# PolyChord/PolyChordLite

Measured on AMD Instinct MI355X. Metric: likelihood evals/sec, 20D Gaussian nlive=2000, higher is better.
Workload: dtype f64; 1 GPU; configs[1]: 20-D Gaussian, nlive=2000, num_repeats=40, one full run per step; batch_chains=1000, parallelism=repeat-sharded x1, mode=one run at a time per GPU; R runs in step: roofline.in_step

## Files before the change

### polychordlite_amd/csrc/pc_contract.hip

```cpp
#include "pc_state.h"
#include "pc_launch.h"
#include <atomic>
#include <cstdlib>
#include <type_traits>

template <int NT>
__device__ __forceinline__ vk_t block_argmin(vk_t v, vk_t *scratch)
{
    v = wave_argmin(v);
    if (NT == 64) return v;
    const int wid = threadIdx.x >> 6;
    if ((threadIdx.x & 63) == 0) scratch[wid] = v;
    __syncthreads();
    vk_t r = scratch[0];
#pragma unroll
    for (int i = 1; i < NT / 64; ++i) r = vk_min(r, scratch[i]);
    __syncthreads();
    return r;
}

struct ConsumeShared {
    double *sL; int *sC; int *sP;
    double *cLogLp, *cLogXp, *cLogZp, *cLogZXp, *cLogZp2, *cLogZpXp, *cLseRef, *cLseSum, *cThr;
    int *cN, *cMinSlot; unsigned *cUid;
// ... 1138 lines not shown
#pragma unroll
                    for (int u = 0; u < 8; ++u) if (u < cnt) dst0[(size_t)idx[u] * nT + e] = v[u];
                }
            }
        }
        return;
    }
    for (int m = 0; m < (nr + 62) / 64; ++m) {
        const unsigned long long mask = S.plan[w].ph_mask[m];
        if (wv == 0 && ((mask >> lane) & 1ull)) {
            const int i = m * 64 + lane, dsti = base + __popcll(mask & ((1ull << lane) - 1ull));
            S.ph_logL[dsti] = S.baby_logL[(size_t)w * nr + i]; S.ph_cuid[dsti] = cuid;
            S.ph_uid[dsti] = ((unsigned long long)batch << 32) | (unsigned)(w * nr + i);
        }
        const unsigned long long mine = mask & (0xFFFFull << (16 * wv));
        const int before = __popcll(mask & ((1ull << (16 * wv)) - 1ull));
        wave_copy_masked(S.babies + ((size_t)w * nr + m * 64) * nT, mine, S.phantom + (size_t)(base + before) * nT, nT, lane);
        base += __popcll(mask);
    }
}
__global__ __launch_bounds__(64 * PC_APPLY_WAVES) void k_apply_dead_ph(PcState S, unsigned batch) { apply_dead_ph_body(S, batch); }
__global__ __launch_bounds__(64 * PC_APPLY_WAVES) void k_apply_dead_ph_many(const PcManyRec *__restrict__ R) { apply_dead_ph_body(pc_many_state(R, blockIdx.y), (unsigned)R[blockIdx.y].ia[PC_REC_I_BATCH]); }

__device__ __forceinline__ void apply_pool_body(const PcState &S, unsigned batch, int nchains)
{
    const PcCtl *ctl = S.ctl;
    const int lane = threadIdx.x & 63, nT = S.nT, nr = S.nr;
    const int item = (int)blockIdx.x * (int)(blockDim.x >> 6) + (int)(threadIdx.x >> 6);
    if (item >= nchains + S.Ncap) return;
    if (item < nchains) {
        const int w = ctl->seg_lo + item;
        if (w > ctl->seg_hi) return;
        const int di = S.plan[w].dead_idx, src = S.plan[w].dead_src;
        if (di >= 0 && src < 0) {
            const double *row = S.babies + ((size_t)(-src - 1) * nr + (nr - 1)) * nT;
            double *dst = S.dead + (size_t)di * nT;
            for (int e = lane; e < nT; e += 64) dst[e] = row[e];
            if (lane == 0) {
                S.dead_logw[di] = S.plan[w].logw; S.dead_postX[di] = S.plan[w].postX + log(S.plan[w].postXs); S.dead_postZ[di] = S.plan[w].postZ;
                S.dead_cuid[di] = S.plan[w].dead_cuid; S.dead_entry[di] = S.plan[-src - 1].contour;
            }
        }
        const int base = S.plan[w].ph_base;
        const unsigned cuid = S.plan[w].ph_cuid;
        const double Lg = S.plan[w].contour;
        for (int i = lane; i < nr; i += 64) {
            const double bl = S.baby_logL[(size_t)w * nr + i];
            S.ph_logL[base + i] = bl; S.ph_cuid[base + i] = ((i < nr - 1) && bl > Lg) ? cuid : PC_CUID_NONE;
            S.ph_uid[base + i] = ((unsigned long long)batch << 32) | (unsigned)(w * nr + i);
        }
        return;
    }
    const int slot = item - nchains;
    const int src = S.slot_src[slot], killer = S.slot_dead[slot];
    if (src < 0 && killer < 0) return;
    double *lrow = S.live + (size_t)slot * nT;
    if (killer >= 0) {
        const int di = S.plan[killer].dead_idx;
        double *dst = S.dead + (size_t)di * nT;
        for (int e = lane; e < nT; e += 64) dst[e] = lrow[e];
        if (lane == 0) {
            S.dead_logw[di] = S.plan[killer].logw; S.dead_postX[di] = S.plan[killer].postX + log(S.plan[killer].postXs); S.dead_postZ[di] = S.plan[killer].postZ;
            S.dead_cuid[di] = S.plan[killer].dead_cuid; S.dead_entry[di] = S.live_entry[slot];
        }
    }
    if (src >= 0) {
        const double *row = S.babies + ((size_t)src * nr + (nr - 1)) * nT;
        double v[4];
#pragma unroll
        for (int q = 0; q < 4; ++q) v[q] = (lane + 64 * q < nT) ? row[lane + 64 * q] : 0.0;
        for (int e = lane + 256; e < nT; e += 64) lrow[e] = row[e];
#pragma unroll
        for (int q = 0; q < 4; ++q) if (lane + 64 * q < nT) lrow[lane + 64 * q] = v[q];
    }
    if (lane == 0) { S.slot_src[slot] = -1; S.slot_dead[slot] = -1; if (src >= 0) S.live_entry[slot] = S.plan[src].contour; }
}
__global__ __launch_bounds__(256) void k_apply_pool(PcState S, unsigned batch, int nchains) { apply_pool_body(S, batch, nchains); }
__global__ __launch_bounds__(256) void k_apply_pool_many(const PcManyRec *R, int nchains) { apply_pool_body(pc_many_state(R, blockIdx.y), (unsigned)R[blockIdx.y].ia[PC_REC_I_BATCH], nchains); }


__device__ __forceinline__ void apply_live_body(const PcState &S)
{
    const int slot = blockIdx.x, lane = threadIdx.x, nT = S.nT, nr = S.nr;
    const int src = S.slot_src[slot];
    if (src < 0) return;
    const double *row = S.babies + ((size_t)src * nr + (nr - 1)) * nT;
    double *dst = S.live + (size_t)slot * nT;
    for (int e = lane; e < nT; e += 64) dst[e] = row[e];
    __syncthreads();
    if (lane == 0) { S.slot_src[slot] = -1; S.live_entry[slot] = S.plan[src].contour; }
}
__global__ __launch_bounds__(64) void k_apply_live(PcState S) { apply_live_body(S); }
__global__ __launch_bounds__(64) void k_apply_live_many(const PcManyRec *__restrict__ R) { apply_live_body(pc_many_state(R, blockIdx.y)); }

__global__ __launch_bounds__(256) void k_install_live(PcState S, const double *rows, int n)
{
    const int tid = threadIdx.x;
    __shared__ vk_t red[4];
    for (int s = tid; s < S.Ncap; s += 256) {
        if (s < n) {
            S.live_logL[s] = rows[(size_t)s * S.nT + S.l0]; S.live_cluster[s] = 0; S.live_pos[s] = s; S.live_entry[s] = S.logzero;
// ... 582 lines not shown
        const size_t sh = consume_lds(S, 1024, cache_x, 0, sgl);
        if (sh > 160 * 1024) return 1;
        pc_need_dyn_lds((const void *)k_consume<1024>, sh);
        hipLaunchKernelGGL((k_consume<1024>), dim3(1), dim3(1024), sh, st, *S, final_mode, cache_x, 0, sgl);
    } else {
        const int sgl = consume_slots_global(S, 64);
        int xr = S->Ncap;
        while (xr > 32 && consume_lds(S, 64, xr, 0, sgl) > 158 * 1024) xr = (xr + 1) / 2;
        const size_t sh = consume_lds(S, 64, xr, 0, sgl);
        if (sh > 160 * 1024) return 1;
        pc_need_dyn_lds((const void *)k_consume<64>, sh);
        hipLaunchKernelGGL((k_consume<64>), dim3(1), dim3(64), sh, st, *S, final_mode, xr, 0, sgl);
    }
    return 0;
}

extern "C" void pc_launch_apply(const PcState *S, unsigned batch, int nchains, hipStream_t st)
{
    if (S->pool) { hipLaunchKernelGGL(k_apply_pool, dim3((nchains + S->Ncap + 3) / 4), dim3(256), 0, st, *S, batch, nchains); return; }
    hipLaunchKernelGGL(k_apply_dead_ph, dim3(nchains), dim3(64 * PC_APPLY_WAVES), 0, st, *S, batch);
    hipLaunchKernelGGL(k_apply_live, dim3(S->Ncap), dim3(64), 0, st, *S);
}

extern "C" int pc_launch_apply_many(const PcState *S, const PcManyRec *dR, int R, unsigned batch, int nchains, hipStream_t st)
{
    if (!S->pool) {
        hipLaunchKernelGGL(k_apply_dead_ph_many, dim3(nchains, R), dim3(64 * PC_APPLY_WAVES), 0, st, dR);
        hipLaunchKernelGGL(k_apply_live_many, dim3(S->Ncap, R), dim3(64), 0, st, dR);
        return 0;
    }
    static const int wpg = std::getenv("PC_APPLY_WAVES") ? std::max(1, std::min(4, std::atoi(std::getenv("PC_APPLY_WAVES")))) : 4;
    hipLaunchKernelGGL(k_apply_pool_many, dim3((nchains + S->Ncap + wpg - 1) / wpg, R), dim3(64 * wpg), 0, st, dR, nchains);
    return 0;
}

extern "C" int pc_launch_clean_many(const PcManyRec *dR, int R, int nblk_max, hipStream_t st)
{
    if (nblk_max < 1) return 1;
    hipLaunchKernelGGL(k_clean_flag_many, dim3(nblk_max, R), dim3(256), 0, st, dR);
    hipLaunchKernelGGL(k_scan_blocks_many, dim3(1, R), dim3(256), 0, st, dR);
    hipLaunchKernelGGL(k_clean_scatter_many, dim3(nblk_max, R), dim3(256), 0, st, dR);
    return 0;
}

extern "C" void pc_launch_install_live(const PcState *S, const double *rows, int n, hipStream_t st)
{
// ... 195 lines not shown
```

### polychordlite_amd/csrc/pc_engine.hip

```cpp
#include "pc_state.h"
#include "pc_resume.h"
#include "pc_prior_table.h"
#include "pc_launch.h"
#include "pc_plan.h"
#include <cstdio>
#include <cstdlib>
#include <cstring>
#include <cstdarg>
#include <cstdint>
#include <new>
#include <cmath>
#include <vector>
#include <memory>
#include <string>
#include <chrono>
#include <algorithm>
#include <map>
#include <unordered_map>
#include <atomic>
#include <mutex>
#include <thread>
#include <functional>
#include <exception>
#include <ucontext.h>
// ... 292 lines not shown
    std::vector<int> cb_idx; std::vector<double> cb_c, cb_t, cb_p, cb_l;
    polychord_dumper_fn dumper = nullptr;
    pchip_update_fn on_update = nullptr; void *hook_user = nullptr;
    long ndiscarded = 0;
    bool resume_static = true; unsigned resume_batch0 = 0;
    bool nph_stale = false;
    std::vector<double> hm_dead, hm_logw; int hm_ndead = 0;
    std::vector<unsigned> hm_cuid;
    std::vector<double> pp_rows, pp_logpost; std::vector<unsigned> pp_cuid; std::vector<unsigned long long> pp_uid; int nd_last_update = 0;
    std::vector<unsigned> split_child, split_parent; std::vector<double> split_logfrac;
    std::vector<double> h_lo, h_hi;
    PcState S{};
    RunBlocks blocks;
    hipStream_t st = nullptr;
    hipStream_t st_copy = nullptr;
    bool st_copy_shared = false;
    hipStream_t st_side = nullptr;
    hipEvent_t ev_main = nullptr;
    static constexpr int RAW_RING = 4;
    struct RawSlot { hipEvent_t ready = nullptr, consumed = nullptr; unsigned batch = 0; int B = 0; bool valid = false, waited = false, used = false; int co_seq = 0; };
    RawSlot ring[RAW_RING];
    int raw_depth = 2;
    double *h_dead = nullptr; size_t h_dead_cap = 0, h_dead_copied = 0;
    PcCtl *h_ctl = nullptr;
    PcCtl *h_note = nullptr;
    unsigned note_seq = 0;
    hipEvent_t ev_apply = nullptr;
    double *raw_buf[RAW_RING] = {nullptr, nullptr, nullptr, nullptr};
    double *ph2 = nullptr, *phL2 = nullptr; unsigned *phC2 = nullptr; unsigned long long *phU2 = nullptr;
    unsigned char *keep = nullptr; int *blk = nullptr, *d_total = nullptr;
    double *psum = nullptr, *mean = nullptr, *pcov = nullptr; int *pcnt = nullptr, *count = nullptr;
    size_t cov_chunks_cap = 0;
    double *upd_part = nullptr, *upd_shift = nullptr; size_t upd_part_cap = 0;
    PcPriorTable ptab; bool have_ptab = false;
    double *d_lo = nullptr, *d_hi = nullptr, *d_invcovT = nullptr, *d_mean = nullptr, *d_src = nullptr;
    double *d_dynL = nullptr; int *d_dynN = nullptr; double *d_logn = nullptr;
    ClusterUpdate<Engine> clus{*this};
    Engine() = default; Engine(const Engine &) = delete; Engine &operator=(const Engine &) = delete;
    std::vector<int> sub_dims; int *c_subdims = nullptr;
    long nsplits = 0; int ncluster_peak = 1;
    bool src_terms = false;
    long path[PCHIP_PATH_COUNT] = {};
    Cohort::Note step_note;
    Timing tm;
    KTimer kt;
    int B = 0, dev = 0;
// ... 581 lines not shown

    PcLaunchTraits launch_traits() const { return PcLaunchTraits{pc_rtc_wanted(&S) != 0, src_terms, S.prior.kind >= PCHIP_PRIOR_TABLE}; }
    PcUpdateFacts update_facts(int nph) const { return PcUpdateFacts{nph > 0, pc_update_fused_ok(&S, h_ctl->ncluster) != 0, h_ctl->ncluster}; }

    void do_update(bool deferred = false)
    {
        tm.updates += deferred ? std::max(1, h_ctl->upd_marks) : 1;
        const bool seq_post = S.seq_mode && (cfg.posteriors || cfg.equals);
        if (plan.ctl == PC_CTL_EARLY) { const int st_keep = h_ctl->status; read_ctl(); h_ctl->status = st_keep; }
        if (!plan.hook_late) call_dumper();
        const int nph = S.pool ? (int)pool_cursor : h_ctl->nphantom;
        const PcUpdateChoice upd = pc_choose_update(plan, update_facts(nph));
        pc_count(path, upd);
        if (upd.kind == PC_UPDATE_FUSED) {
            const size_t need = (size_t)pc_update_fused_blocks(&S, nph) * pc_update_fused_entries(&S);
            if (need > upd_part_cap) { blocks.release(upd_part); upd_part_cap = 2 * need; upd_part = blocks.dev<double>(upd_part_cap); }
            if (!upd_shift) {
                upd_shift = blocks.dev<double>(S.D);
                std::vector<double> half(S.D, 0.5);
                HIPCHK(hipMemcpyAsync(upd_shift, half.data(), sizeof(double) * S.D, hipMemcpyHostToDevice, st));
                HIPCHK(hipStreamSynchronize(st));
            }
            hipEvent_t e0 = kt.begin(KT_CLEAN);
            (void)stage(rec_update(S, keep, blk, d_total, ph2, phL2, phC2, phU2, upd_part, upd_shift, co ? pc_update_fused_grid(&S, nph, deferred ? 1 : 0) : 0, deferred, nph));
            kt.end(KT_CLEAN, e0);
            if (upd.need_count) {
                std::vector<int> tot;
                fetch(tot, (const int *)d_total, 1);
                fetch_wait();
                const int total = tot[0];
                h_ctl->nphantom = total;
                if (seq_post) seq_consume((unsigned long long)(nph - total));
            } else nph_stale = true;
            if (!S.pool) { std::swap(S.phantom, ph2); std::swap(S.ph_logL, phL2); std::swap(S.ph_cuid, phC2); std::swap(S.ph_uid, phU2); }
            write_resume();
            return;
        }
        if (deferred) engine_fail(PC_RC_DEVICE, "deferred update without the fused update path");
        hipEvent_t e0 = kt.begin(KT_CLEAN);
        if (co && nph <= 0) { direct_op(); pc_launch_clean(&S, nph, keep, blk, d_total, ph2, phL2, phC2, phU2, nullptr, st); }
        else (void)stage(rec_compact(S, keep, blk, d_total, ph2, phL2, phC2, phU2, nph));
        kt.end(KT_CLEAN, e0);
        if (plan.hook_late) { collect_phantom_posteriors(nph); call_dumper(); }
        const bool need_count = upd.need_count, ctl_late = upd.ctl == PC_CTL_LATE;
        int total = nph;
        std::vector<int> tot, cn;
        if (need_count) {
// ... 438 lines not shown
        bool resumed = false;
        if (cfg.resume_read) {
            if (FILE *probe = std::fopen(cfg.resume_read, "r")) {
                std::fclose(probe);
                PcResume rs; std::string err;
                if (!pc_resume_read(cfg.resume_read, rs, err) || !import_resume(rs, err)) { std::fprintf(stderr, "polychord_hip: %s\n", err.c_str()); return 6; }
                resumed = true;
                int ntot = 0;
                for (int v : rs.nlive) ntot += v;
                if (ntot > cfg.nlive && rs.ncluster == 1) { pc_count(path, PcTrimLive{}); pc_launch_consume(&S, 2, 0, st); read_ctl(); ntot = cfg.nlive; }
                resume_static = (ntot == cfg.nlive);
                resume_batch0 = (unsigned)rs.ndead;
            }
        }
        if (!resumed) { if (callback_mode) generate_live_callback(); else generate_live(); }
        if (stop.load(std::memory_order_relaxed)) return 5;
        if (cb_auto_batch && !(cb_eval_seconds >= 0.0 && cb_eval_seconds < 2e-6)) { B = B_small; S.B = B; }
        r_t1 = clk::now();
        r_batch = resume_batch0;
        r_sort_valid = false;
        r_nursery_left = 0;
        make_plan();
        S.defer_update = plan.defer ? 1 : 0; S.pool = plan.pool ? 1 : 0;
        if (S.pool) {
            pool_cursor = h_ctl->nphantom;
            if (g_cap_phantoms.load() <= 0) {
                size_t free_b = 0, total_b = 0;
                (void)hipMemGetInfo(&free_b, &total_b);
                const double need = 2.0 * 2.0 * (double)S.Pcap * ((double)S.nT * 8.0 + 24.0);
                if (need < 0.4 * (double)free_b) grow_phantoms(2LL * S.Pcap);
            }
        }
        r_rc = 0;
        return -1;
    }

    void make_plan()
    {
        const int nprior0 = cfg.nprior <= 0 ? cfg.nlive : cfg.nprior;
        PcRunFacts f{};
        f.ablate = cfg.ablate; f.force_general = cfg.force_general;
        f.fixed_nlive = (cfg.n_nlives == 0) && (nprior0 >= cfg.nlive) && resume_static;
        f.par_fits = pc_par_fits(&S) != 0; f.fast_fits = pc_fast_fits(&S) != 0; f.fused_fits_one = pc_update_fused_ok(&S, 1) != 0;
        f.clustering = cfg.do_clustering != 0; f.boost = cfg.boost_posterior != 0.0;
        f.dumper = dumper != nullptr; f.on_update = on_update != nullptr; f.resume_write = cfg.resume_write != nullptr;
        f.seq_mode = S.seq_mode != 0; f.posteriors = cfg.posteriors || cfg.equals;
// ... 184 lines not shown
                sort_valid = false;
                if (ch.want_nn) { co->rec(rec_nn(S, nursery_left)); S.nn_valid = 1; }
                co->rec(rec_sort(S));
                co->rec(rec_consume_cl(S, h_ctl->ncluster > 64));
                break;
            case PC_CONTRACT_CL: case PC_CONTRACT_GENERAL: {
                sort_valid = false;
                if (co) co->flush();
                bool sorted_now = false;
                if (presorted) { HIPCHK(hipStreamWaitEvent(st, ev_presort_b, 0)); sorted_now = fresh_nursery; presorted = false; }
                if (ch.want_nn) {
                    if (!sorted_now) sorted_now = pc_launch_sort_live(&S, st) == 0;
                    pc_launch_nn_lists(&S, nursery_left, sorted_now ? 1 : 0, st);
                    S.nn_valid = 1;
                }
                if (ch.kind == PC_CONTRACT_CL) rc2 = (sorted_now ? 0 : pc_launch_sort_live(&S, st)) || pc_launch_consume_cl(&S, h_ctl->ncluster, st);
                else rc2 = pc_launch_consume(&S, 0, (h_ctl->ncluster > 1) ? 1 : 0, st);
                break;
            }
            }
            if (rc2) { std::fprintf(stderr, "polychord_hip: nlive too large for the LDS-resident contraction\n"); r_rc = 4; return false; }
            kt.end(KT_CONSUME, e2);
            hipEvent_t e3 = kt.begin(KT_APPLY);
            (void)stage(rec_apply(S, batch - 1, B));
            kt.end(KT_APPLY, e3);
            if (st_side) { RawSlot &rs = ring[batch % raw_depth]; if (rs.valid && rs.batch == batch && !rs.waited) { HIPCHK(hipStreamWaitEvent(st, rs.ready, 0)); rs.waited = true; } }
            r_fresh = fresh_nursery;
            ready_spins = 0;
        }
        return true;
    }

    bool finish_may_wait() const
    {
        const bool upd = h_ctl->status == PC_ST_UPDATE || (h_ctl->upd_pending && h_ctl->status == PC_ST_RUNNING);
        return upd && pc_choose_update(plan, update_facts(1)).may_wait;
    }
    bool round_finish()
    {
        unsigned &batch = r_batch; int &nursery_left = r_nursery_left; const bool fresh_nursery = r_fresh;
        (void)batch;
        {
            if (fresh_nursery && h_ctl->status == PC_ST_DONE && h_ctl->i_nursery == B) tm.batches--;
            nursery_left = h_ctl->i_nursery;
            tally_grades();
            tm.rounds++;
// ... 722 lines not shown
```

### polychordlite_amd/csrc/pc_launch.h

```cpp
#pragma once
#include "pc_state.h"
#include "../../include/polychord_hip.h"
#include <cstddef>

extern "C" int pc_rtc_source_sums(int id);
extern "C" long pc_rtc_source_quad(int id);

static inline size_t pc_quad_lds(const PcState *S)
{
    if (S->like.kind != PC_LIKE_SOURCE) return 0;
    const long n = pc_rtc_source_quad(S->src_id);
    return n > 0 ? sizeof(double) * 2 * (size_t)((n + 1) & ~1L) : 0;
}

static inline int pc_slice_phi_lds(const PcState *S)
{
    const size_t sh0 = sizeof(double) * ((size_t)S->D + S->nr) + 16, tb = sizeof(double) * (size_t)S->nr * (S->D + 1);
    const size_t sums = S->like.kind == PC_LIKE_SOURCE ? sizeof(double) * (size_t)S->nr * (size_t)pc_rtc_source_sums(S->src_id) : 0;
    return (S->nDer > 0 && sh0 + tb + sums + pc_quad_lds(S) <= 48 * 1024) ? 1 : 0;
}

extern "C" {

void pc_abi_set_last_error(const char *msg);
void pc_launch_slice_tick(const PcState *S, unsigned batch, int nchains, void *cs, double *x0s, int *decks, double *prop, const double *ev_logL,
                          const double *ev_theta, const double *ev_phi, int first, double *prop_host, int *need_host, hipStream_t st);
size_t pc_chain_state_size(void);
int pc_launch_killoff_cl(const PcState *S, int nc, hipStream_t st);
int pc_consume_cl_fits(const PcState *S, int nc);
int pc_consume_clp_fits(const PcState *S, int nc);
int pc_launch_consume_cl_many(const PcState *S, const PcManyRec *dR, int R, int wide, hipStream_t st);
int pc_launch_consume_cl(const PcState *S, int nc, hipStream_t st);
int pc_launch_knn_cluster_sub(const int *d_desc, int nb, int mmax, const double *Sm, const int *pool, int *knn, int *labels, int *out, hipStream_t st);
int pc_launch_knn_cluster_sub_many(const PcManyRec *dR, int R, int nb_max, int mmax, hipStream_t st);
void pc_launch_remap_chains(const PcState *S, const int *map, int nold, int n, hipStream_t st);
void pc_launch_shift_mats(const PcState *S, int p, int nc, hipStream_t st);
int pc_launch_knn_cluster_batch(const PcState *S, const int *h_desc, const int *d_desc, int nd, double *Sm, int *knn, int *labels, int *out, const int *dims, int ndims, hipStream_t st);
int pc_launch_knn_cluster_batch_dev(const PcState *S, const int *d_desc, int nd, int nmax, double *Sm, int *knn, int *labels, int *out, const int *dims, int ndims, hipStream_t st);
int pc_launch_knn_cluster_batch_many(const PcState *S, const PcManyRec *dR, int R, int nd_max, int nmax, int any_sub, hipStream_t st);
void pc_launch_rebuild(const PcState *S, int nc, hipStream_t st);
void pc_launch_ph_rehome(const PcState *S, int nph, int nc, const unsigned *old_uids, int nold_uids, int *counts, hipStream_t st);
void pc_launch_nn_lists(const PcState *S, int nleft, int use_rank, hipStream_t st);
int pc_launch_nn_lists_many(const PcState *S, const PcManyRec *dR, int R, int nleft_max, int use_rank, hipStream_t st);
int pc_launch_consume(const PcState *S, int final_mode, int wide, hipStream_t st);
void pc_launch_apply(const PcState *S, unsigned batch, int nchains, hipStream_t st);
int pc_launch_apply_many(const PcState *S, const PcManyRec *dR, int R, unsigned batch, int nchains, hipStream_t st);
int pc_launch_clean_many(const PcManyRec *dR, int R, int nblk_max, hipStream_t st);
void pc_launch_install_live(const PcState *S, const double *rows, int n, hipStream_t st);
void pc_launch_clean(const PcState *S, int nph, unsigned char *keep, int *blk, int *d_total, double *ph2, double *phL2, unsigned *phC2, unsigned long long *phU2, int *dst_index, hipStream_t st);
void pc_launch_reset_thresholds(const PcState *S, hipStream_t st);
int pc_launch_reset_thresholds_many(const PcState *S, const PcManyRec *dR, int R, hipStream_t st);
int pc_cov_nchunk(const PcState *S, int nph);
int pc_launch_covmats(const PcState *S, int nph, int nc, double *psum, int *pcnt, double *mean, int *count, double *pcov, hipStream_t st);
void pc_launch_scan_blocks(int *blk, int nblk, int *total, int *total2, hipStream_t st);
void pc_launch_chol_only(const PcState *S, const double *ncov, const int *count, hipStream_t st);
void pc_launch_init_state(const PcState *S, double logzero, hipStream_t st);
int pc_post_blocks(void);
void pc_launch_post_moments(const PcState *S, int nd, double *pmax, double *part, hipStream_t st);
void pc_prepare_streams(int dev, int want);
void *pc_cache_dev_alloc(size_t bytes);
void pc_cache_dev_free(void *p);
void *pc_cache_host_alloc(size_t bytes);
void pc_cache_host_free(void *p);
int pc_run_many(const pchip_settings *s, const pchip_like *like, const pchip_prior *prior, int nseeds, const int *seeds, int device, int max_in_flight, pchip_result *results);
void *pc_source_batch_open(int handle, int device, int nDims, int nDerived, polychord_prior_fn prior);
void pc_source_batch_eval(void *user, int n, int nDims, int nDerived, const double *cube, double *theta, double *phi, double *logL);
void pc_source_batch_close(void *user);
void pc_batch_callback_get(polychord_batch_fn *fn, void **user);
// ... 27 lines not shown
int pc_launch_slice_step(const PcState *S, const PcManyRec *dR, int R, int nchains, int fused, hipStream_t st);
int pc_launch_nhats_many(const PcState *S, const PcManyRec *dR, int R, int nchains, hipStream_t st);
int pc_launch_slice(const PcState *S, unsigned batch, int nchains, hipStream_t st);
int pc_launch_prior_transform(const PcState *S, int n, const double *cubes, double *thetas, hipStream_t st);
int pc_launch_source_eval(const PcState *S, int n, const double *thetas, double *logL, double *phi, hipStream_t st);
int pc_launch_source_prior_eval(const PcState *S, int n, const double *cubes, double *thetas, hipStream_t st);
int pc_launch_max_rank(const PcState *S, int n, const double *rows, double *val, hipStream_t st);
int pc_launch_maximise(const PcState *S, int nprob, const double *in, const int *hdr, long long max_iter, double *out, long long *outi, hipStream_t st);
int pc_max_choose_simplex(int nDims, int nTotal, double logzero, const double *live, const int *cluster, int nlive, const double *vals,
                          double *simplex, double *f);
void pc_maximum_alloc(pchip_maximum *m, int nDims, int nDerived);
int pc_bases_t_ok(const PcState *S);
int pc_launch_bases_t(const PcState *S, unsigned batch, int nchains, hipStream_t st);
int pc_launch_bases_t_many(const PcState *S, const PcManyRec *dR, int R, unsigned batch, int nchains, hipStream_t st);
int pc_slice_t_ok(const PcState *S, int ncluster);
int pc_launch_slice_t(const PcState *S, unsigned batch, int nchains, hipStream_t st);
int pc_launch_slice_t_many(const PcState *S, const PcManyRec *dR, int R, unsigned batch, int nchains, hipStream_t st);
int pc_update_fused_ok(const PcState *S, int nc);
int pc_update_fused_blocks(const PcState *S, int nph);
int pc_update_fused_entries(const PcState *S);
#define PC_UPD_CTR_INTS 2048
void pc_launch_update_fused(const PcState *S, int nph, unsigned char *keep, int *blk, int *d_total, double *ph2, double *phL2, unsigned *phC2,
                            unsigned long long *phU2, double *part, double *shift, int deferred, hipStream_t st);
int pc_update_fused_grid(const PcState *S, int nph, int deferred);
int pc_launch_update_fused_many(const PcState *S, const PcManyRec *dR, int R, int nblk_max, int G, int deferred, hipStream_t st);

}
```

### polychordlite_amd/csrc/pc_state.h

```cpp
#pragma once
#include "pc_dev.h"

enum { PC_ST_RUNNING = 0, PC_ST_DONE = 1, PC_ST_UPDATE = 2, PC_ST_ERROR = 4 };
enum { PC_ERR_NONE = 0, PC_ERR_PHANTOM_CAP = 1, PC_ERR_DEAD_CAP = 2, PC_ERR_CLUSTER_CAP = 3, PC_ERR_NOSLOT = 4 };

enum { PC_ABL_FUNCTOR = 1 << 0, PC_ABL_NO_POOL = 1 << 1, PC_ABL_NO_DEFER = 1 << 2, PC_ABL_NO_FUSED_UPDATE = 1 << 3, PC_ABL_PAIR_SCANS = 1 << 4,
       PC_ABL_CONSUME_GENERAL = 1 << 5, PC_ABL_SLICE_LANE = 1 << 6, PC_ABL_BASES_PACKED = 1 << 7, PC_ABL_CL_END_AT_DEATH = 1 << 8,
       PC_ABL_KILLOFF_GENERAL = 1 << 9, PC_ABL_CONSUME_CL_SERIAL = 1 << 10, PC_ABL_RETIRED_11 = 1 << 11, PC_ABL_RETIRED_12 = 1 << 12,
       PC_ABL_NO_HELPER = 1 << 13, PC_ABL_QC_BY_CHAIN = 1 << 14, PC_ABL_RTC_BUILTINS = 1 << 15, PC_ABL_UPDATE_CHAIN = 1 << 16, PC_ABL_TRACE_CHOL = 1 << 30 };

#define PC_MASK_WORDS 16

struct PcCtl {
    int status;
    int error;
    int i_nursery;
    int admin_epoch;
    int failures;
    int ncluster;
    int ncluster_dead;
    int ndead;
    int nphantom;
    int seg_hi, seg_lo;
    int cluster_deleted;
    unsigned batch_id;
    unsigned next_cluster_uid;
    long long nlike;
    long long niter;
    long long nlike_device;
    long long nlike_failed;
    double logZ, logZ2;
    double logX_last_update;
// ... 222 lines not shown
```

### polychordlite_amd/csrc/pc_update.hip

```cpp
#include "pc_state.h"
#include "pc_launch.h"
#include <atomic>
#include <cstdio>
#include <cstdlib>

#define UPD_ROWS 256
#define UPD_NT 256

__device__ __forceinline__ void upd_stage_masked(const double *src0, unsigned long long mask, unsigned long long mmask, double *dst,
                                                 double *tile, int TS, const double *sh, int D, int nT, int lane)
{
    const int ne = dst ? nT : D + 1;
    int n = 0;
    while (mask) {
        int idx[16], cnt = 0;
#pragma unroll
        for (int u = 0; u < 16; ++u) {
            idx[u] = 0;
            if (mask) { idx[u] = __ffsll((long long)mask) - 1; mask &= mask - 1; cnt = u + 1; }
        }
        for (int e = lane; e < ne; e += 64) {
            double v[16];
#pragma unroll
            for (int u = 0; u < 16; ++u) if (u < cnt) v[u] = (e < nT) ? src0[(size_t)idx[u] * nT + e] : 0.0;
            if (dst) {
#pragma unroll
                for (int u = 0; u < 16; ++u) if (u < cnt) dst[(size_t)(n + u) * nT + e] = v[u];
            }
            if (e <= D) {
                const double s = e < D ? sh[e] : 0.0;
#pragma unroll
                for (int u = 0; u < 16; ++u)
                    if (u < cnt && ((mmask >> idx[u]) & 1ull))
                        tile[(size_t)__popcll(mmask & ((1ull << idx[u]) - 1ull)) * TS + e] = e < D ? v[u] - s : 1.0;
            }
        }
        n += cnt;
    }
}

template <typename T> __device__ __forceinline__ void upd_store_wt(T *p, T v) { __hip_atomic_store(p, v, __ATOMIC_RELAXED, __HIP_MEMORY_SCOPE_AGENT); }
__device__ __forceinline__ void upd_flag_body(const PcState &S, int nph, unsigned char *keep, int *blk_count, int def, int nblk)
{
    const int tid = threadIdx.x, lane = tid & 63, wv = tid >> 6;
    const int sb = blockIdx.x * 4 + wv;
    if (sb >= nblk) return;
    const unsigned uid0 = S.cl_uid[0];
    const double thr = def ? S.ctl->upd_thr : S.death_thr[0];
    const bool pool = S.pool;
    const int tmark = (pool && def) ? S.ctl->upd_tmark : 0x7fffffff, nph0u = (pool && def) ? S.ctl->upd_nph0 : 0x7fffffff;
    const int T = (pool && def) ? S.ctl->upd_T : 0, nr = S.nr;
    const int j0 = sb * UPD_ROWS + 4 * lane;
    const bool full = j0 + 3 < nph;
    unsigned cu[4] = {PC_CUID_NONE, PC_CUID_NONE, PC_CUID_NONE, PC_CUID_NONE};
    double ll[4] = {0.0, 0.0, 0.0, 0.0};
    if (full) {
        const uint4 c = *(const uint4 *)(S.ph_cuid + j0);
        const double2 a = *(const double2 *)(S.ph_logL + j0), b2 = *(const double2 *)(S.ph_logL + j0 + 2);
        cu[0] = c.x; cu[1] = c.y; cu[2] = c.z; cu[3] = c.w; ll[0] = a.x; ll[1] = a.y; ll[2] = b2.x; ll[3] = b2.y;
    } else {
        for (int u = 0; u < 4; ++u) if (j0 + u < nph) { cu[u] = S.ph_cuid[j0 + u]; ll[u] = S.ph_logL[j0 + u]; }
    }
    unsigned kb = 0; bool wr = false; int cnt = 0;
#pragma unroll
    for (int u = 0; u < 4; ++u) {
        const int j = j0 + u;
        bool k = false, km = false;
        if (j < nph) {
            k = (cu[u] == uid0) && !(ll[u] < thr);
            if (pool) {
                if (!k && cu[u] == uid0) { cu[u] = PC_CUID_NONE; wr = true; }
                km = k && (j < nph0u || T - 1 - (j - nph0u) / nr < tmark);
            }
            kb |= (unsigned)((k ? 1 : 0) | (km ? 2 : 0)) << (8 * u);
        }
        cnt += __popcll(__ballot(pool ? km : k));
    }
    if (full) {
        *(unsigned *)(keep + j0) = kb;
        if (wr) *(uint4 *)(S.ph_cuid + j0) = make_uint4(cu[0], cu[1], cu[2], cu[3]);
    } else {
        for (int u = 0; u < 4; ++u) if (j0 + u < nph) { keep[j0 + u] = (unsigned char)((kb >> (8 * u)) & 0xFFu); if (wr) S.ph_cuid[j0 + u] = cu[u]; }
    }
    if (lane == 0) upd_store_wt(blk_count + sb, cnt);
}
__global__ __launch_bounds__(UPD_NT) void k_upd_flag(PcState S, int nph, unsigned char *keep, int *blk_count, int def, int nblk) { upd_flag_body(S, nph, keep, blk_count, def, nblk); }
__global__ __launch_bounds__(UPD_NT) void k_upd_flag_many(const PcManyRec *R, int def) { const PcManyView r = pc_many_view(R, blockIdx.y); if ((int)blockIdx.x * 4 >= r.ia[PC_REC_I_BLOCKS]) return; upd_flag_body(r.S, r.ia[PC_REC_I_ROWS], (unsigned char *)r.p[PC_REC_KEEP], (int *)r.p[PC_REC_BLK], def, r.ia[PC_REC_I_BLOCKS]); }

__device__ __forceinline__ bool upd_ticket_last(int *ctr, int n, int *last_s)
{
    asm volatile("s_waitcnt vmcnt(0)" ::: "memory");
    __syncthreads();
    if (threadIdx.x == 0) {
        const int t = __hip_atomic_fetch_add(ctr, 1, __ATOMIC_RELAXED, __HIP_MEMORY_SCOPE_AGENT);
        const int last = t == n - 1;
        if (last) {
            __builtin_amdgcn_fence(__ATOMIC_ACQUIRE, "agent");
            asm volatile("s_waitcnt vmcnt(0)" ::: "memory");
            __hip_atomic_store(ctr, 0, __ATOMIC_RELAXED, __HIP_MEMORY_SCOPE_AGENT);
        }
        *last_s = last;
    }
    __syncthreads();
    return *last_s != 0;
}
#define UPD_TICKET_FLAG 1
#define UPD_TICKET_FINAL 2
#define UPD_TICKET_GROUP 16

#define UPD_SELF_BLOCKS 4096
__global__ __launch_bounds__(UPD_NT) void k_upd_flag_scan(PcState S, int nph, unsigned char *keep, int *blk, int def, int nblk, int *ctr)
{
    __shared__ int last_s, wsum[4];
    upd_flag_body(S, nph, keep, blk, def, nblk);
    if (!upd_ticket_last(ctr + UPD_TICKET_FLAG, (int)gridDim.x, &last_s)) return;
    const int tid = threadIdx.x, lane = tid & 63, wv = tid >> 6, i0 = 16 * tid;
    int c[16], s = 0;
#pragma unroll
    for (int u = 0; u < 16; ++u) { c[u] = (i0 + u < nblk) ? blk[i0 + u] : 0; s += c[u]; }
    int inc = s;
#pragma unroll
    for (int o = 1; o < 64; o <<= 1) { const int t = __shfl_up(inc, o); if (lane >= o) inc += t; }
    if (lane == 63) wsum[wv] = inc;
    __syncthreads();
    int run = inc - s;
    for (int x = 0; x < wv; ++x) run += wsum[x];
#pragma unroll
    for (int u = 0; u < 16; ++u) { if (i0 + u < nblk) blk[i0 + u] = run; run += c[u]; }
    if (tid == UPD_NT - 1) ctr[0] = run;
}


__global__ __launch_bounds__(1024) void k_upd_scan(int *cnt, int n, int *total)
{
    __shared__ int wsum[16];
    __shared__ int carry_s;
    const int tid = threadIdx.x, lane = tid & 63, wv = tid >> 6;
// ... 499 lines not shown
}

static int upd_grid(const PcState *S, int nph, int deferred)
{
    const int nblk = (nph + UPD_ROWS - 1) / UPD_ROWS, nlb = (S->Ncap + UPD_ROWS - 1) / UPD_ROWS, ndb = deferred ? (S->B + UPD_ROWS - 1) / UPD_ROWS : 0;
    static const int cap_env = std::getenv("PC_UPD_GRID") ? std::atoi(std::getenv("PC_UPD_GRID")) : 0;
    const int cap = cap_env > 0 ? cap_env : (S->D < 32 ? 384 : 512);
    if (S->pool) { const int nch = (nph + 63) / 64; return (nch < cap ? (nch > 0 ? nch : 1) : cap) + nlb + ndb; }
    const int total = nblk + nlb + ndb;
    return total < cap ? total : cap;
}

extern "C" int pc_update_fused_ok(const PcState *S, int nc) { return nc == 1 && S->D <= 128; }
extern "C" int pc_update_fused_blocks(const PcState *S, int nph)
{
    const int G = upd_grid(S, nph, 1), E = pc_update_fused_entries(S);
    return G + (G + UPD_FOLD - 1) / UPD_FOLD + (S->D * S->D + 2 + E - 1) / E;
}
extern "C" int pc_update_fused_entries(const PcState *S) { const int e = S->D * (S->D + 1) / 2 + S->D + 1; return (e + 31) & ~31; }

extern "C" void pc_launch_update_fused(const PcState *S, int nph, unsigned char *keep, int *blk, int *d_total, double *ph2, double *phL2,
                                       unsigned *phC2, unsigned long long *phU2, double *part, double *shift, int deferred, hipStream_t st)
{
    const int D = S->D, nblk = (nph + UPD_ROWS - 1) / UPD_ROWS, nlb = (S->Ncap + UPD_ROWS - 1) / UPD_ROWS, E = pc_update_fused_entries(S);
    const int ndb = deferred ? (S->B + UPD_ROWS - 1) / UPD_ROWS : 0;
    const int NTv = (D + 1 + 15) / 16, TSv = NTv <= 2 ? 16 * NTv + 1 : 16 * NTv + ((NTv & 1) ? 0 : 16), CAPv = NTv <= 2 ? 128 : 64;
    const int G = upd_grid(S, nph, deferred), ng = (G + UPD_FOLD - 1) / UPD_FOLD;
    double *part2 = part + (size_t)G * E;
    size_t shw = sizeof(double) * ((size_t)CAPv * TSv + D);
    if (NTv <= 2 && shw < sizeof(double) * (size_t)(4 * 3 * 256)) shw = sizeof(double) * (size_t)(4 * 3 * 256);
    if (S->pool && nblk <= UPD_SELF_BLOCKS && UPD_TICKET_GROUP + ng <= PC_UPD_CTR_INTS && (S->ablate & PC_ABL_UPDATE_CHAIN)) {
        int *ctr = d_total;
        hipLaunchKernelGGL(k_upd_flag_scan, dim3((nblk + 3) / 4), dim3(UPD_NT), 0, st, *S, nph, keep, blk, deferred, nblk, ctr);
#define UPDC_LAUNCH(NT) { \
        pc_need_dyn_lds((const void *)k_upd_chain<NT>, shw); \
        hipLaunchKernelGGL((k_upd_chain<NT>), dim3(G), dim3(256), shw, st, *S, nph, nblk, (const unsigned char *)keep, (const int *)blk, shift, part, E, deferred, nlb, ndb, ctr); }
        switch (NTv) { case 1: UPDC_LAUNCH(1) break; case 2: UPDC_LAUNCH(2) break; case 3: UPDC_LAUNCH(3) break; case 4: UPDC_LAUNCH(4) break;
                       case 5: UPDC_LAUNCH(5) break; case 6: UPDC_LAUNCH(6) break; case 7: UPDC_LAUNCH(7) break; case 8: UPDC_LAUNCH(8) break;
                       default: UPDC_LAUNCH(9) break; }
#undef UPDC_LAUNCH
        if (D < 32) return;
    } else {
        hipLaunchKernelGGL(k_upd_flag, dim3((nblk + 3) / 4), dim3(UPD_NT), 0, st, *S, nph, keep, blk, deferred, nblk);
        if (!S->pool) pc_launch_scan_blocks(blk, nblk, d_total, &S->ctl->nphantom, st);
        else if (nblk <= UPD_SELF_BLOCKS && !std::getenv("PC_UPD_SCAN_LAUNCH"))
            hipLaunchKernelGGL(k_upd_index_self, dim3((nblk + 15) / 16), dim3(UPD_IDX_NT), 0, st, nph, (const unsigned char *)keep, (const int *)blk, nblk, (int *)phC2, d_total);
        else {
            hipLaunchKernelGGL(k_upd_scan, dim3(1), dim3(1024), 0, st, blk, nblk, d_total);
            hipLaunchKernelGGL(k_upd_index, dim3(nblk), dim3(UPD_NT), 0, st, nph, (const unsigned char *)keep, (const int *)blk, (int *)phC2);
        }
        int devi = 0; (void)hipGetDevice(&devi); devi &= 63;
#define UPDG_LAUNCH(NT) { \
            pc_need_dyn_lds((const void *)k_upd_gather<NT, false>, shw); \
                              pc_need_dyn_lds((const void *)k_upd_gather<NT, true>, shw); \
             \
            if (S->pool) hipLaunchKernelGGL((k_upd_gather<NT, true>), dim3(G), dim3(256), shw, st, *S, nph, nblk, (const unsigned char *)keep, (const int *)blk, \
                               ph2, phL2, phC2, phU2, (const int *)phC2, (const int *)d_total, (const double *)shift, part, E, deferred, nlb, ndb); \
            else hipLaunchKernelGGL((k_upd_gather<NT, false>), dim3(G), dim3(256), shw, st, *S, nph, nblk, (const unsigned char *)keep, (const int *)blk, \
                               ph2, phL2, phC2, phU2, (const int *)nullptr, (const int *)nullptr, (const double *)shift, part, E, deferred, nlb, ndb); }
        switch (NTv) { case 1: UPDG_LAUNCH(1) break; case 2: UPDG_LAUNCH(2) break; case 3: UPDG_LAUNCH(3) break; case 4: UPDG_LAUNCH(4) break;
                       case 5: UPDG_LAUNCH(5) break; case 6: UPDG_LAUNCH(6) break; case 7: UPDG_LAUNCH(7) break; case 8: UPDG_LAUNCH(8) break;
                       default: UPDG_LAUNCH(9) break; }
#undef UPDG_LAUNCH
    }
    hipLaunchKernelGGL(k_upd_fold, dim3(ng), dim3(256), 0, st, (const double *)part, G, E, part2);
    if (D < 32) { hipLaunchKernelGGL(k_upd_final, dim3(1), dim3(256), 0, st, *S, ng, (const double *)part2, E, shift, deferred); return; }
// ... 31 lines not shown
```

Measured before the change: 1.340 billion likelihood evals/s.

## Fuse update flag pass into the pool apply kernel launch

Adds a combined kernel that runs the deferred-update flag pass in some blocks and the pool apply (dead/live copies) in the others. For the chain's phantom rows, the flag blocks read baby logL and plan data directly and write the phantom entries, so the apply kernel no longer writes them. The next update then skips its separate flag launch. This removes a kernel launch and one pass over the phantom arrays, at the cost of more complex region-aware flag logic and host-side state that tracks whether flags are already valid.

```diff
diff --git a/polychordlite_amd/csrc/pc_contract.hip b/polychordlite_amd/csrc/pc_contract.hip
--- a/polychordlite_amd/csrc/pc_contract.hip
+++ b/polychordlite_amd/csrc/pc_contract.hip
@@ -1,5 +1,6 @@
 #include "pc_state.h"
 #include "pc_launch.h"
+#include "pc_upd_flag.h"
 #include <atomic>
 #include <cstdlib>
 #include <type_traits>
@@ -1184,11 +1185,12 @@
 __global__ __launch_bounds__(64 * PC_APPLY_WAVES) void k_apply_dead_ph(PcState S, unsigned batch) { apply_dead_ph_body(S, batch); }
 __global__ __launch_bounds__(64 * PC_APPLY_WAVES) void k_apply_dead_ph_many(const PcManyRec *__restrict__ R) { apply_dead_ph_body(pc_many_state(R, blockIdx.y), (unsigned)R[blockIdx.y].ia[PC_REC_I_BATCH]); }
 
-__device__ __forceinline__ void apply_pool_body(const PcState &S, unsigned batch, int nchains)
+template <bool IDS>
+__device__ __forceinline__ void apply_pool_body(const PcState &S, unsigned batch, int nchains, int wg)
 {
     const PcCtl *ctl = S.ctl;
     const int lane = threadIdx.x & 63, nT = S.nT, nr = S.nr;
-    const int item = (int)blockIdx.x * (int)(blockDim.x >> 6) + (int)(threadIdx.x >> 6);
+    const int item = wg * (int)(blockDim.x >> 6) + (int)(threadIdx.x >> 6);
     if (item >= nchains + S.Ncap) return;
     if (item < nchains) {
         const int w = ctl->seg_lo + item;
@@ -1203,6 +1205,7 @@
                 S.dead_cuid[di] = S.plan[w].dead_cuid; S.dead_entry[di] = S.plan[-src - 1].contour;
             }
         }
+        if (!IDS) return;
         const int base = S.plan[w].ph_base;
         const unsigned cuid = S.plan[w].ph_cuid;
         const double Lg = S.plan[w].contour;
@@ -1237,8 +1240,13 @@
     }
     if (lane == 0) { S.slot_src[slot] = -1; S.slot_dead[slot] = -1; if (src >= 0) S.live_entry[slot] = S.plan[src].contour; }
 }
-__global__ __launch_bounds__(256) void k_apply_pool(PcState S, unsigned batch, int nchains) { apply_pool_body(S, batch, nchains); }
-__global__ __launch_bounds__(256) void k_apply_pool_many(const PcManyRec *R, int nchains) { apply_pool_body(pc_many_state(R, blockIdx.y), (unsigned)R[blockIdx.y].ia[PC_REC_I_BATCH], nchains); }
+__global__ __launch_bounds__(256) void k_apply_pool(PcState S, unsigned batch, int nchains) { apply_pool_body<true>(S, batch, nchains, (int)blockIdx.x); }
+__global__ __launch_bounds__(256) void k_apply_pool_many(const PcManyRec *R, int nchains) { apply_pool_body<true>(pc_many_state(R, blockIdx.y), (unsigned)R[blockIdx.y].ia[PC_REC_I_BATCH], nchains, (int)blockIdx.x); }
+__global__ __launch_bounds__(256) void k_apply_pool_flag(PcState S, unsigned batch, int nchains, int nb_flag, int nph, unsigned char *keep, int *blk, int nblk)
+{
+    if ((int)blockIdx.x >= nb_flag) { apply_pool_body<false>(S, batch, nchains, (int)blockIdx.x - nb_flag); return; }
+    upd_flag_body<true>(S, nph, keep, blk, 1, nblk, (int)blockIdx.x * 4 + (int)(threadIdx.x >> 6), batch);
+}
 
 
 __device__ __forceinline__ void apply_live_body(const PcState &S)
@@ -1867,6 +1875,12 @@
     hipLaunchKernelGGL(k_apply_live, dim3(S->Ncap), dim3(64), 0, st, *S);
 }
 
+extern "C" void pc_launch_apply_flag(const PcState *S, unsigned batch, int nchains, int nph, unsigned char *keep, int *blk, hipStream_t st)
+{
+    const int nb_apply = (nchains + S->Ncap + 3) / 4, nblk = (nph + UPD_ROWS - 1) / UPD_ROWS, nb_flag = (nblk + 3) / 4;
+    hipLaunchKernelGGL(k_apply_pool_flag, dim3(nb_flag + nb_apply), dim3(256), 0, st, *S, batch, nchains, nb_flag, nph, keep, blk, nblk);
+}
+
 extern "C" int pc_launch_apply_many(const PcState *S, const PcManyRec *dR, int R, unsigned batch, int nchains, hipStream_t st)
 {
     if (!S->pool) {
diff --git a/polychordlite_amd/csrc/pc_engine.hip b/polychordlite_amd/csrc/pc_engine.hip
--- a/polychordlite_amd/csrc/pc_engine.hip
+++ b/polychordlite_amd/csrc/pc_engine.hip
@@ -338,6 +338,7 @@
     RawSlot ring[RAW_RING];
     int raw_depth = 2;
     double *h_dead = nullptr; size_t h_dead_cap = 0, h_dead_copied = 0;
+    bool r_flagged = false; int r_flag_nph = 0; unsigned char *r_flag_keep = nullptr; int *r_flag_blk = nullptr;
     PcCtl *h_ctl = nullptr;
     PcCtl *h_note = nullptr;
     unsigned note_seq = 0;
@@ -965,7 +966,11 @@
                 HIPCHK(hipStreamSynchronize(st));
             }
             hipEvent_t e0 = kt.begin(KT_CLEAN);
+            if (!co && deferred && r_flagged && r_flag_nph == nph && r_flag_keep == keep && r_flag_blk == blk)
+                pc_launch_update_fused_at(&S, nph, keep, blk, d_total, ph2, phL2, phC2, phU2, upd_part, upd_shift, 1, 1, st);
+            else
             (void)stage(rec_update(S, keep, blk, d_total, ph2, phL2, phC2, phU2, upd_part, upd_shift, co ? pc_update_fused_grid(&S, nph, deferred ? 1 : 0) : 0, deferred, nph));
+            r_flagged = false;
             kt.end(KT_CLEAN, e0);
             if (upd.need_count) {
                 std::vector<int> tot;
@@ -1450,6 +1455,7 @@
         r_nursery_left = 0;
         make_plan();
         S.defer_update = plan.defer ? 1 : 0; S.pool = plan.pool ? 1 : 0;
+        r_flagged = false;
         if (S.pool) {
             pool_cursor = h_ctl->nphantom;
             if (g_cap_phantoms.load() <= 0) {
@@ -1680,6 +1686,12 @@
             if (rc2) { std::fprintf(stderr, "polychord_hip: nlive too large for the LDS-resident contraction\n"); r_rc = 4; return false; }
             kt.end(KT_CONSUME, e2);
             hipEvent_t e3 = kt.begin(KT_APPLY);
+            r_flagged = !co && S.pool && S.defer_update && plan.fused_update && ch.kind == PC_CONTRACT_PAR && pool_cursor >= 1 && keep && blk &&
+                        !(S.ablate & (PC_ABL_FLAG_LAUNCH | PC_ABL_UPDATE_CHAIN));
+            if (r_flagged) {
+                r_flag_nph = (int)pool_cursor; r_flag_keep = keep; r_flag_blk = blk;
+                pc_launch_apply_flag(&S, batch - 1, B, r_flag_nph, keep, blk, st);
+            } else
             (void)stage(rec_apply(S, batch - 1, B));
             kt.end(KT_APPLY, e3);
             if (st_side) { RawSlot &rs = ring[batch % raw_depth]; if (rs.valid && rs.batch == batch && !rs.waited) { HIPCHK(hipStreamWaitEvent(st, rs.ready, 0)); rs.waited = true; } }
diff --git a/polychordlite_amd/csrc/pc_launch.h b/polychordlite_amd/csrc/pc_launch.h
--- a/polychordlite_amd/csrc/pc_launch.h
+++ b/polychordlite_amd/csrc/pc_launch.h
@@ -44,6 +44,7 @@
 int pc_launch_nn_lists_many(const PcState *S, const PcManyRec *dR, int R, int nleft_max, int use_rank, hipStream_t st);
 int pc_launch_consume(const PcState *S, int final_mode, int wide, hipStream_t st);
 void pc_launch_apply(const PcState *S, unsigned batch, int nchains, hipStream_t st);
+void pc_launch_apply_flag(const PcState *S, unsigned batch, int nchains, int nph, unsigned char *keep, int *blk, hipStream_t st);
 int pc_launch_apply_many(const PcState *S, const PcManyRec *dR, int R, unsigned batch, int nchains, hipStream_t st);
 int pc_launch_clean_many(const PcManyRec *dR, int R, int nblk_max, hipStream_t st);
 void pc_launch_install_live(const PcState *S, const double *rows, int n, hipStream_t st);
@@ -117,6 +118,8 @@
 #define PC_UPD_CTR_INTS 2048
 void pc_launch_update_fused(const PcState *S, int nph, unsigned char *keep, int *blk, int *d_total, double *ph2, double *phL2, unsigned *phC2,
                             unsigned long long *phU2, double *part, double *shift, int deferred, hipStream_t st);
+void pc_launch_update_fused_at(const PcState *S, int nph, unsigned char *keep, int *blk, int *d_total, double *ph2, double *phL2, unsigned *phC2,
+                               unsigned long long *phU2, double *part, double *shift, int deferred, int flagged, hipStream_t st);
 int pc_update_fused_grid(const PcState *S, int nph, int deferred);
 int pc_launch_update_fused_many(const PcState *S, const PcManyRec *dR, int R, int nblk_max, int G, int deferred, hipStream_t st);
 
diff --git a/polychordlite_amd/csrc/pc_state.h b/polychordlite_amd/csrc/pc_state.h
--- a/polychordlite_amd/csrc/pc_state.h
+++ b/polychordlite_amd/csrc/pc_state.h
@@ -7,7 +7,8 @@
 enum { PC_ABL_FUNCTOR = 1 << 0, PC_ABL_NO_POOL = 1 << 1, PC_ABL_NO_DEFER = 1 << 2, PC_ABL_NO_FUSED_UPDATE = 1 << 3, PC_ABL_PAIR_SCANS = 1 << 4,
        PC_ABL_CONSUME_GENERAL = 1 << 5, PC_ABL_SLICE_LANE = 1 << 6, PC_ABL_BASES_PACKED = 1 << 7, PC_ABL_CL_END_AT_DEATH = 1 << 8,
        PC_ABL_KILLOFF_GENERAL = 1 << 9, PC_ABL_CONSUME_CL_SERIAL = 1 << 10, PC_ABL_RETIRED_11 = 1 << 11, PC_ABL_RETIRED_12 = 1 << 12,
-       PC_ABL_NO_HELPER = 1 << 13, PC_ABL_QC_BY_CHAIN = 1 << 14, PC_ABL_RTC_BUILTINS = 1 << 15, PC_ABL_UPDATE_CHAIN = 1 << 16, PC_ABL_TRACE_CHOL = 1 << 30 };
+       PC_ABL_NO_HELPER = 1 << 13, PC_ABL_QC_BY_CHAIN = 1 << 14, PC_ABL_RTC_BUILTINS = 1 << 15, PC_ABL_UPDATE_CHAIN = 1 << 16, PC_ABL_FLAG_LAUNCH = 1 << 17,
+       PC_ABL_TRACE_CHOL = 1 << 30 };
 
 #define PC_MASK_WORDS 16
 
diff --git a/polychordlite_amd/csrc/pc_upd_flag.h b/polychordlite_amd/csrc/pc_upd_flag.h
--- /dev/null
+++ b/polychordlite_amd/csrc/pc_upd_flag.h
@@ -0,0 +1,91 @@
+#pragma once
+#include "pc_state.h"
+
+#define UPD_ROWS 256
+#define UPD_NT 256
+
+template <typename T> __device__ __forceinline__ void upd_store_wt(T *p, T v) { __hip_atomic_store(p, v, __ATOMIC_RELAXED, __HIP_MEMORY_SCOPE_AGENT); }
+template <bool REGION>
+__device__ __forceinline__ void upd_flag_body(const PcState &S, int nph, unsigned char *keep, int *blk_count, int def, int nblk, int sb, unsigned batch = 0u)
+{
+    const int lane = threadIdx.x & 63;
+    if (sb >= nblk) return;
+    const int nr = S.nr;
+    const int j0 = sb * UPD_ROWS + 4 * lane;
+    bool pending = true;
+    int r_lo = 0, r_hi = 0;
+    if (REGION) {
+        const PcCtl *ctl = S.ctl;
+        pending = ctl->upd_pending != 0;
+        r_lo = S.pool_base + ctl->seg_lo * nr; r_hi = S.pool_base + (ctl->seg_hi + 1) * nr;
+        if (!pending && !(sb * UPD_ROWS < r_hi && sb * UPD_ROWS + UPD_ROWS > r_lo)) return;
+    }
+    const unsigned uid0 = S.cl_uid[0];
+    const double thr = def ? S.ctl->upd_thr : S.death_thr[0];
+    const bool pool = S.pool;
+    const int tmark = (pool && def) ? S.ctl->upd_tmark : 0x7fffffff, nph0u = (pool && def) ? S.ctl->upd_nph0 : 0x7fffffff;
+    const int T = (pool && def) ? S.ctl->upd_T : 0;
+    const bool full = j0 + 3 < nph;
+    const bool mixed = REGION && j0 < r_hi && j0 + 3 >= r_lo;
+    unsigned cu[4] = {PC_CUID_NONE, PC_CUID_NONE, PC_CUID_NONE, PC_CUID_NONE};
+    double ll[4] = {0.0, 0.0, 0.0, 0.0};
+    if (mixed) {
+        int w = 0, i = 0; bool in = false; double Lg = 0.0; unsigned pc = PC_CUID_NONE;
+#pragma unroll
+        for (int u = 0; u < 4; ++u) {
+            const int j = j0 + u;
+            if (j >= nph) continue;
+            if (j >= r_lo && j < r_hi) {
+                if (!in) { const int q = j - S.pool_base; w = q / nr; i = q - w * nr; in = true; Lg = S.plan[w].contour; pc = S.plan[w].ph_cuid; }
+                else if (++i == nr) { i = 0; ++w; Lg = S.plan[w].contour; pc = S.plan[w].ph_cuid; }
+                const double bl = S.baby_logL[j - S.pool_base];
+                ll[u] = bl; cu[u] = ((i < nr - 1) && bl > Lg) ? pc : PC_CUID_NONE;
+            } else { cu[u] = S.ph_cuid[j]; ll[u] = S.ph_logL[j]; }
+        }
+    } else if (full) {
+        const uint4 c = *(const uint4 *)(S.ph_cuid + j0);
+        const double2 a = *(const double2 *)(S.ph_logL + j0), b2 = *(const double2 *)(S.ph_logL + j0 + 2);
+        cu[0] = c.x; cu[1] = c.y; cu[2] = c.z; cu[3] = c.w; ll[0] = a.x; ll[1] = a.y; ll[2] = b2.x; ll[3] = b2.y;
+    } else {
+        for (int u = 0; u < 4; ++u) if (j0 + u < nph) { cu[u] = S.ph_cuid[j0 + u]; ll[u] = S.ph_logL[j0 + u]; }
+    }
+    unsigned kb = 0; bool wr = false; int cnt = 0;
+    if (pending) {
+#pragma unroll
+        for (int u = 0; u < 4; ++u) {
+            const int j = j0 + u;
+            bool k = false, km = false;
+            if (j < nph) {
+                k = (cu[u] == uid0) && !(ll[u] < thr);
+                if (pool) {
+                    if (!k && cu[u] == uid0) { cu[u] = PC_CUID_NONE; wr = true; }
+                    km = k && (j < nph0u || T - 1 - (j - nph0u) / nr < tmark);
+                }
+                kb |= (unsigned)((k ? 1 : 0) | (km ? 2 : 0)) << (8 * u);
+            }
+            cnt += __popcll(__ballot(pool ? km : k));
+        }
+        if (full) *(unsigned *)(keep + j0) = kb;
+        else for (int u = 0; u < 4; ++u) if (j0 + u < nph) keep[j0 + u] = (unsigned char)((kb >> (8 * u)) & 0xFFu);
+    }
+    if (mixed && full && j0 >= r_lo && j0 + 3 < r_hi) {
+        const unsigned long long u0 = ((unsigned long long)batch << 32) | (unsigned)(j0 - S.pool_base);
+        *(double2 *)(S.ph_logL + j0) = make_double2(ll[0], ll[1]); *(double2 *)(S.ph_logL + j0 + 2) = make_double2(ll[2], ll[3]);
+        *(uint4 *)(S.ph_cuid + j0) = make_uint4(cu[0], cu[1], cu[2], cu[3]);
+        *(ulonglong2 *)(S.ph_uid + j0) = make_ulonglong2(u0, u0 + 1); *(ulonglong2 *)(S.ph_uid + j0 + 2) = make_ulonglong2(u0 + 2, u0 + 3);
+    } else if (mixed) {
+#pragma unroll
+        for (int u = 0; u < 4; ++u) {
+            const int j = j0 + u;
+            if (j >= nph) continue;
+            if (j >= r_lo && j < r_hi) {
+                S.ph_logL[j] = ll[u]; S.ph_cuid[j] = cu[u];
+                S.ph_uid[j] = ((unsigned long long)batch << 32) | (unsigned)(j - S.pool_base);
+            } else if (wr) S.ph_cuid[j] = cu[u];
+        }
+    } else if (wr) {
+        if (full) *(uint4 *)(S.ph_cuid + j0) = make_uint4(cu[0], cu[1], cu[2], cu[3]);
+        else for (int u = 0; u < 4; ++u) if (j0 + u < nph) S.ph_cuid[j0 + u] = cu[u];
+    }
+    if (pending && lane == 0) upd_store_wt(blk_count + sb, cnt);
+}
diff --git a/polychordlite_amd/csrc/pc_update.hip b/polychordlite_amd/csrc/pc_update.hip
--- a/polychordlite_amd/csrc/pc_update.hip
+++ b/polychordlite_amd/csrc/pc_update.hip
@@ -1,11 +1,10 @@
 #include "pc_state.h"
 #include "pc_launch.h"
+#include "pc_upd_flag.h"
 #include <atomic>
 #include <cstdio>
 #include <cstdlib>
 
-#define UPD_ROWS 256
-#define UPD_NT 256
 
 __device__ __forceinline__ void upd_stage_masked(const double *src0, unsigned long long mask, unsigned long long mmask, double *dst,
                                                  double *tile, int TS, const double *sh, int D, int nT, int lane)
@@ -39,53 +38,8 @@
     }
 }
 
-template <typename T> __device__ __forceinline__ void upd_store_wt(T *p, T v) { __hip_atomic_store(p, v, __ATOMIC_RELAXED, __HIP_MEMORY_SCOPE_AGENT); }
-__device__ __forceinline__ void upd_flag_body(const PcState &S, int nph, unsigned char *keep, int *blk_count, int def, int nblk)
-{
-    const int tid = threadIdx.x, lane = tid & 63, wv = tid >> 6;
-    const int sb = blockIdx.x * 4 + wv;
-    if (sb >= nblk) return;
-    const unsigned uid0 = S.cl_uid[0];
-    const double thr = def ? S.ctl->upd_thr : S.death_thr[0];
-    const bool pool = S.pool;
-    const int tmark = (pool && def) ? S.ctl->upd_tmark : 0x7fffffff, nph0u = (pool && def) ? S.ctl->upd_nph0 : 0x7fffffff;
-    const int T = (pool && def) ? S.ctl->upd_T : 0, nr = S.nr;
-    const int j0 = sb * UPD_ROWS + 4 * lane;
-    const bool full = j0 + 3 < nph;
-    unsigned cu[4] = {PC_CUID_NONE, PC_CUID_NONE, PC_CUID_NONE, PC_CUID_NONE};
-    double ll[4] = {0.0, 0.0, 0.0, 0.0};
-    if (full) {
-        const uint4 c = *(const uint4 *)(S.ph_cuid + j0);
-        const double2 a = *(const double2 *)(S.ph_logL + j0), b2 = *(const double2 *)(S.ph_logL + j0 + 2);
-        cu[0] = c.x; cu[1] = c.y; cu[2] = c.z; cu[3] = c.w; ll[0] = a.x; ll[1] = a.y; ll[2] = b2.x; ll[3] = b2.y;
-    } else {
-        for (int u = 0; u < 4; ++u) if (j0 + u < nph) { cu[u] = S.ph_cuid[j0 + u]; ll[u] = S.ph_logL[j0 + u]; }
-    }
-    unsigned kb = 0; bool wr = false; int cnt = 0;
-#pragma unroll
-    for (int u = 0; u < 4; ++u) {
-        const int j = j0 + u;
-        bool k = false, km = false;
-        if (j < nph) {
-            k = (cu[u] == uid0) && !(ll[u] < thr);
-            if (pool) {
-                if (!k && cu[u] == uid0) { cu[u] = PC_CUID_NONE; wr = true; }
-                km = k && (j < nph0u || T - 1 - (j - nph0u) / nr < tmark);
-            }
-            kb |= (unsigned)((k ? 1 : 0) | (km ? 2 : 0)) << (8 * u);
-        }
-        cnt += __popcll(__ballot(pool ? km : k));
-    }
-    if (full) {
-        *(unsigned *)(keep + j0) = kb;
-        if (wr) *(uint4 *)(S.ph_cuid + j0) = make_uint4(cu[0], cu[1], cu[2], cu[3]);
-    } else {
-        for (int u = 0; u < 4; ++u) if (j0 + u < nph) { keep[j0 + u] = (unsigned char)((kb >> (8 * u)) & 0xFFu); if (wr) S.ph_cuid[j0 + u] = cu[u]; }
-    }
-    if (lane == 0) upd_store_wt(blk_count + sb, cnt);
-}
-__global__ __launch_bounds__(UPD_NT) void k_upd_flag(PcState S, int nph, unsigned char *keep, int *blk_count, int def, int nblk) { upd_flag_body(S, nph, keep, blk_count, def, nblk); }
-__global__ __launch_bounds__(UPD_NT) void k_upd_flag_many(const PcManyRec *R, int def) { const PcManyView r = pc_many_view(R, blockIdx.y); if ((int)blockIdx.x * 4 >= r.ia[PC_REC_I_BLOCKS]) return; upd_flag_body(r.S, r.ia[PC_REC_I_ROWS], (unsigned char *)r.p[PC_REC_KEEP], (int *)r.p[PC_REC_BLK], def, r.ia[PC_REC_I_BLOCKS]); }
+__global__ __launch_bounds__(UPD_NT) void k_upd_flag(PcState S, int nph, unsigned char *keep, int *blk_count, int def, int nblk) { upd_flag_body<false>(S, nph, keep, blk_count, def, nblk, (int)blockIdx.x * 4 + (int)(threadIdx.x >> 6)); }
+__global__ __launch_bounds__(UPD_NT) void k_upd_flag_many(const PcManyRec *R, int def) { const PcManyView r = pc_many_view(R, blockIdx.y); if ((int)blockIdx.x * 4 >= r.ia[PC_REC_I_BLOCKS]) return; upd_flag_body<false>(r.S, r.ia[PC_REC_I_ROWS], (unsigned char *)r.p[PC_REC_KEEP], (int *)r.p[PC_REC_BLK], def, r.ia[PC_REC_I_BLOCKS], (int)blockIdx.x * 4 + (int)(threadIdx.x >> 6)); }
 
 __device__ __forceinline__ bool upd_ticket_last(int *ctr, int n, int *last_s)
 {
@@ -112,7 +66,7 @@
 __global__ __launch_bounds__(UPD_NT) void k_upd_flag_scan(PcState S, int nph, unsigned char *keep, int *blk, int def, int nblk, int *ctr)
 {
     __shared__ int last_s, wsum[4];
-    upd_flag_body(S, nph, keep, blk, def, nblk);
+    upd_flag_body<false>(S, nph, keep, blk, def, nblk, (int)blockIdx.x * 4 + (int)(threadIdx.x >> 6));
     if (!upd_ticket_last(ctr + UPD_TICKET_FLAG, (int)gridDim.x, &last_s)) return;
     const int tid = threadIdx.x, lane = tid & 63, wv = tid >> 6, i0 = 16 * tid;
     int c[16], s = 0;
@@ -658,6 +612,11 @@
 extern "C" void pc_launch_update_fused(const PcState *S, int nph, unsigned char *keep, int *blk, int *d_total, double *ph2, double *phL2,
                                        unsigned *phC2, unsigned long long *phU2, double *part, double *shift, int deferred, hipStream_t st)
 {
+    pc_launch_update_fused_at(S, nph, keep, blk, d_total, ph2, phL2, phC2, phU2, part, shift, deferred, 0, st);
+}
+extern "C" void pc_launch_update_fused_at(const PcState *S, int nph, unsigned char *keep, int *blk, int *d_total, double *ph2, double *phL2,
+                                          unsigned *phC2, unsigned long long *phU2, double *part, double *shift, int deferred, int flagged, hipStream_t st)
+{
     const int D = S->D, nblk = (nph + UPD_ROWS - 1) / UPD_ROWS, nlb = (S->Ncap + UPD_ROWS - 1) / UPD_ROWS, E = pc_update_fused_entries(S);
     const int ndb = deferred ? (S->B + UPD_ROWS - 1) / UPD_ROWS : 0;
     const int NTv = (D + 1 + 15) / 16, TSv = NTv <= 2 ? 16 * NTv + 1 : 16 * NTv + ((NTv & 1) ? 0 : 16), CAPv = NTv <= 2 ? 128 : 64;
@@ -677,7 +636,7 @@
 #undef UPDC_LAUNCH
         if (D < 32) return;
     } else {
-        hipLaunchKernelGGL(k_upd_flag, dim3((nblk + 3) / 4), dim3(UPD_NT), 0, st, *S, nph, keep, blk, deferred, nblk);
+        if (!(flagged && S->pool && deferred)) hipLaunchKernelGGL(k_upd_flag, dim3((nblk + 3) / 4), dim3(UPD_NT), 0, st, *S, nph, keep, blk, deferred, nblk);
         if (!S->pool) pc_launch_scan_blocks(blk, nblk, d_total, &S->ctl->nphantom, st);
         else if (nblk <= UPD_SELF_BLOCKS && !std::getenv("PC_UPD_SCAN_LAUNCH"))
             hipLaunchKernelGGL(k_upd_index_self, dim3((nblk + 15) / 16), dim3(UPD_IDX_NT), 0, st, nph, (const unsigned char *)keep, (const int *)blk, nblk, (int *)phC2, d_total);
```

Measured after the change: 1.361 billion likelihood evals/s, median of 6. 1.5% higher.
